# Xiugapurin/Etude

Measured on NVIDIA B200. Metric: extract_throughput_audio_seconds_per_second, higher is better.
Workload: dtype bf16

## Files before the change

etude_b200/csrc/api.cu:

```cuda
#include <algorithm>
#include <cmath>
#include <cstdarg>
#include <cstdio>
#include <cstdlib>
#include <cstring>
#include <string>
#include <map>
#include <vector>

#include "../../include/etude_b200.h"
#include "../../include/etude_b200_kernels.h"
#include "attention2.cuh"
#include "attention4.cuh"
#include "attn_qkv.cuh"
#include "attn_pair.cuh"
#include "chain3.cuh"
#include "embed2.cuh"
#include "gemm.cuh"
#include "logmel.cuh"
#include "logmel2.cuh"
#include "ingest.cuh"
#include "notes.cuh"
#include "pairmma.cuh"
#ifdef ETUDE_DEV_BUILD
// ... 476 lines not shown
    set_smem((const void*)gemm_tcgen05_kernel<256, EPI_BIAS>, gemm_smem_bytes<256, EPI_BIAS>());
    set_smem((const void*)gemm_tcgen05_kernel<256, EPI_BIAS_RELU>, gemm_smem_bytes<256, EPI_BIAS_RELU>());
    set_smem((const void*)gemm_tcgen05_kernel<256, EPI_RESID_LN>, gemm_smem_bytes<256, EPI_RESID_LN>());
#endif
    set_smem((const void*)gemm_tcgen05_kernel<144, EPI_HEADS>, gemm_smem_bytes<144, EPI_HEADS>());
    set_smem((const void*)gemm_bstat_kernel, kGemmBsSmemBytes);
    set_smem((const void*)attention2_kernel<256>, kAttn2SmemBytes);
    set_smem((const void*)attention2_kernel<96>, kAttn2SmemBytes);
    set_smem((const void*)attention4_kernel<128>, kAttn4SmemBytes);
    set_smem((const void*)attention4_kernel<96>, kAttn4SmemBytes);
#ifdef ETUDE_HAVE_ATTN_QKV_CTA1
    set_smem((const void*)attn_qkv_kernel, kAttnQkvSmemBytes);
#endif
    set_smem((const void*)attn_pair_kernel, kAttnPairSmemBytes);
    set_smem((const void*)chain3_kernel<true>, kChain3SmemBytes);
    set_smem((const void*)chain3_kernel<false>, kChain3SmemBytes);
    set_smem((const void*)embed2_kernel, kEmbed2SmemBytes);
    set_smem((const void*)ingest_pcm_kernel, kIngestSmemBudget);
    auto max_smem_carveout = [&](const void* fn) {
        if (e == cudaSuccess) e = cudaFuncSetAttribute(fn, cudaFuncAttributePreferredSharedMemoryCarveout, (int)cudaSharedmemCarveoutMaxShared);
    };
    for (const void* fn : {(const void*)ingest_pcm_kernel, (const void*)notes_transpose_kernel, (const void*)notes_scan_kernel, (const void*)notes_walk_kernel,
                           (const void*)notes_compact_kernel, (const void*)notes_bases_kernel, (const void*)notes_rank_kernel})
        max_smem_carveout(fn);
    set_smem((const void*)logmel2_kernel, kLogmel2SmemBytes);
    if (e != cudaSuccess) status = fail("cudaFuncSetAttribute failed: %s", cudaGetErrorString(e));
    return status;
}

static int num_sms_cached() {
    static int n = 0;
    if (!n) {
        int dev = 0;
        cudaGetDevice(&dev);
        cudaDeviceGetAttribute(&n, cudaDevAttrMultiProcessorCount, dev);
        if (n <= 0) n = 148;
    }
    return n;
}

struct GemmIO {
    __nv_bfloat16* out_bf16 = nullptr;
    int ld_out = 0;
    float* out_f32 = nullptr;
    const float* resid = nullptr;
    int64_t resid_rows = 0;
};

template <int BLOCK_N, int EPI>
static int launch_gemm(const void* a, const void* w, GemmParams p, const GemmIO& io, cudaStream_t st, Profile* prof = nullptr) {
    if (p.K % kBlockK) return fail("gemm: K=%d not a multiple of %d", p.K, kBlockK);
    if (p.N % BLOCK_N) return fail("gemm: N=%d not a multiple of the tile width %d", p.N, BLOCK_N);
    CUtensorMap ta, tb, tob, tof, tr;
    if (make_tmap(&ta, a, (uint64_t)p.M, (uint64_t)p.K, (uint64_t)p.K, kBlockM)) return -1;
    if (make_tmap(&tb, w, (uint64_t)p.N, (uint64_t)p.K, (uint64_t)p.K, BLOCK_N)) return -1;
    tob = ta; tof = ta; tr = ta;
    if (EPI == EPI_BIAS || EPI == EPI_BIAS_RELU) {
        if (!io.out_bf16) return fail("gemm: missing bf16 output");
        if (make_tmap_ex(&tob, io.out_bf16, (uint64_t)p.M, (uint64_t)p.N, (uint64_t)io.ld_out, 32, 64, 2)) return -1;
    } else if (EPI == EPI_RESID_LN) {
        if (!io.out_bf16 || !io.out_f32 || !io.resid) return fail("gemm: LayerNorm epilogue needs out_bf16, out_f32 and resid");
        if (make_tmap_ex(&tob, io.out_bf16, (uint64_t)p.M, 256, 256, 32, 32, 2)) return -1;
        if (make_tmap_ex(&tof, io.out_f32, (uint64_t)p.M, 256, 256, 32, 32, 4)) return -1;
        if (make_tmap_ex(&tr, io.resid, (uint64_t)io.resid_rows, 256, 256, 32, 32, 4)) return -1;
    }
    p.num_m_tiles = (p.M + kBlockM - 1) / kBlockM;
    p.num_n_tiles = p.N / BLOCK_N;
    const int tiles = p.num_m_tiles * p.num_n_tiles;
    const int grid = std::min(tiles, num_sms_cached());
    const int cls = EPI == EPI_RESID_LN ? PC_GEMM_LN : (EPI == EPI_HEADS ? PC_GEMM_HEADS : PC_GEMM_BIAS);
    const int n_alg = EPI == EPI_HEADS ? 3 + kVel : p.N;
    cudaEvent_t ev = prof ? prof->begin(cls, st, 2.0 * p.M * (double)n_alg * p.K, 0.0) : nullptr;
    gemm_tcgen05_kernel<BLOCK_N, EPI><<<grid, kGemmThreads, gemm_smem_bytes<BLOCK_N, EPI>(), st>>>(ta, tb, tob, tof, tr, p);
    if (prof) prof->end(ev, st);
    CUDA_OK(cudaGetLastError());
    {
        char what[96];
        snprintf(what, sizeof what, "gemm epi=%d M=%d N=%d K=%d", EPI, p.M, p.N, p.K);
        if (debug_sync(what, st)) return -1;
    }
    return 0;
}

static int launch_gemm_bstat(const void* a, const void* w, const float* bias, int M, int N, __nv_bfloat16* out, cudaStream_t st, Profile* prof) {
    if (N % 256) return fail("gemm_bstat: N=%d not a multiple of 256", N);
    CUtensorMap ta, tb, to;
    if (make_tmap(&ta, a, (uint64_t)M, 256, 256, kBlockM)) return -1;
    if (make_tmap(&tb, w, (uint64_t)N, 256, 256, 256)) return -1;
    if (make_tmap_ex(&to, out, (uint64_t)M, (uint64_t)N, (uint64_t)N, 32, 64, 2)) return -1;
    GemmParams p{};
    p.M = M; p.N = N; p.K = 256; p.bias = bias;
    p.num_m_tiles = (M + kBlockM - 1) / kBlockM;
    p.num_n_tiles = N / 256;
    const int grid = std::max(1, num_sms_cached() / p.num_n_tiles) * p.num_n_tiles;
    cudaEvent_t ev = prof ? prof->begin(PC_GEMM_BIAS, st, 2.0 * M * (double)N * 256.0, 0.0) : nullptr;
    gemm_bstat_kernel<<<grid, kBsThreads, kGemmBsSmemBytes, st>>>(ta, tb, to, p);
    if (prof) prof->end(ev, st);
    CUDA_OK(cudaGetLastError());
    {
        char what[96];
        snprintf(what, sizeof what, "gemm_bstat M=%d N=%d", M, N);
        if (debug_sync(what, st)) return -1;
    }
    return 0;
}

static int gemm_bias(const void* a, const Linear& L, int M, __nv_bfloat16* out, cudaStream_t st, Profile* prof) {
    if (L.k != 256 || L.n % 256 != 0) return fail("gemm_bias: unsupported projection shape N=%d K=%d", L.n, L.k);
    return launch_gemm_bstat(a, L.w, L.b, M, L.n, out, st, prof);
}

static long long* g_chain_trace = nullptr;

static int launch_attention(const void* q, int64_t q_rows, int q_ld, int q_col0, int q_seq_stride, const void* kv, int kv_ld,
                            int k_col0, int v_col0, int n_seq, int Lq, int Lk, __nv_bfloat16* out, float* probs, cudaStream_t st,
                            Profile* prof = nullptr) {
    const int gen = probs != nullptr ? 2 : 4;
    Attn2Params p{};
    int kb;
    if (Lk == 88) kb = 96;
    else if (Lk == 128) kb = 128;
    else if (Lk == 256 || Lk == 512) kb = gen == 4 ? 128 : 256;
    else return fail("attention: unsupported key length %d", Lk);
    if (Lq > 512 || Lq < 1) return fail("attention: unsupported query length %d", Lq);
    p.Lq = Lq; p.Lk = Lk; p.n_items = n_seq * kHeads; p.q_seq_stride = q_seq_stride;
    p.QT = (Lq + 127) / 128;
    p.NKV = (Lk + kb - 1) / kb;
    if (probs && (p.NKV != 1 || kb == 128)) return fail("attention: the probabilities output is built for one block of 88 or 256 keys");
    if (gen == 4 ? (2 * p.NKV > kA4KvSlots) : (2 * p.NKV + 1 > kA2KvSlots || p.NKV > 2))
        return fail("attention: %d KV blocks exceed the smem ring", p.NKV);
    p.q_col0 = q_col0; p.k_col0 = k_col0; p.v_col0 = v_col0;
    p.out = out; p.probs = probs;
    p.trace = g_chain_trace;
    p.scale_log2e = 1.4426950408889634f / 8.0f;
    CUtensorMap tq, tkv;
    if (make_tmap(&tq, q, (uint64_t)q_rows, (uint64_t)q_ld, (uint64_t)q_ld, 128)) return -1;
    if (make_tmap(&tkv, kv, (uint64_t)n_seq * Lk, (uint64_t)kv_ld, (uint64_t)kv_ld, kb)) return -1;
    const int grid = std::min(p.n_items, num_sms_cached());
    cudaEvent_t ev = prof ? prof->begin(PC_ATTN, st, 4.0 * n_seq * kHeads * (double)Lq * Lk * kHeadDim, 0.0) : nullptr;
    if (gen == 2) {
        if (kb == 256) attention2_kernel<256><<<grid, kAttn2Threads, kAttn2SmemBytes, st>>>(tq, tkv, p);
        else attention2_kernel<96><<<grid, kAttn2Threads, kAttn2SmemBytes, st>>>(tq, tkv, p);
    } else {
        if (kb == 128) attention4_kernel<128><<<grid, kAttn4Threads, kAttn4SmemBytes, st>>>(tq, tkv, p);
        else attention4_kernel<96><<<grid, kAttn4Threads, kAttn4SmemBytes, st>>>(tq, tkv, p);
    }
    if (prof) prof->end(ev, st);
    CUDA_OK(cudaGetLastError());
    {
        char what[96];
        snprintf(what, sizeof what, "attention gen%d n_seq=%d Lq=%d Lk=%d", gen, n_seq, Lq, Lk);
        if (debug_sync(what, st)) return -1;
    }
    return 0;
}

#ifdef ETUDE_DEV_BUILD
extern "C" int etude_debug_mma_bench(int mode, int n, int iters, int n_bufs, int grid, int64_t* host_out) {
    long long* d = nullptr;
    CUDA_OK(cudaMalloc((void**)&d, 16));
    CUDA_OK(cudaFuncSetAttribute((const void*)mma_bench_kernel, cudaFuncAttributeMaxDynamicSharedMemorySize, 210 * 1024));
    mma_bench_kernel<<<grid, 128, 210 * 1024>>>(mode, n, iters, n_bufs, d);
    CUDA_OK(cudaDeviceSynchronize());
    CUDA_OK(cudaMemcpy(host_out, d, 16, cudaMemcpyDeviceToHost));
    cudaFree(d);
    return 0;
}

extern "C" int etude_debug_mma_mix(int ts, int iters, int n_ld, int st_too, int grid, int64_t* host_out) {
    long long* d = nullptr;
    CUDA_OK(cudaMalloc((void**)&d, 32));
    CUDA_OK(cudaMemset(d, 0, 32));
    CUDA_OK(cudaFuncSetAttribute((const void*)mma_mix_kernel, cudaFuncAttributeMaxDynamicSharedMemorySize, 140 * 1024));
    mma_mix_kernel<<<grid, 768, 140 * 1024>>>(ts, iters, n_ld, st_too, d);
    CUDA_OK(cudaDeviceSynchronize());
    CUDA_OK(cudaMemcpy(host_out, d, 16, cudaMemcpyDeviceToHost));
    cudaFree(d);
    return 0;
}

extern "C" int etude_debug_tmem_bench(int mode, int n_warps, int iters, int grid, int64_t* host_out) {
    long long* d = nullptr;
    CUDA_OK(cudaMalloc((void**)&d, 32));
    CUDA_OK(cudaMemset(d, 0, 32));
    tmem_bench_kernel<<<grid, 32 * n_warps>>>(mode, iters, d, reinterpret_cast<float*>(d + 2));
    CUDA_OK(cudaDeviceSynchronize());
    CUDA_OK(cudaMemcpy(host_out, d, 8, cudaMemcpyDeviceToHost));
    cudaFree(d);
    return 0;
}

extern "C" int etude_debug_chain_trace(int enable, int64_t* host_out, int n_values) {
    const size_t bytes = (size_t)64 * 1024;
    if (host_out && g_chain_trace) {
        CUDA_OK(cudaDeviceSynchronize());
// ... 796 lines not shown
```

etude_b200/csrc/attn_qkv.cuh:

```cuda
#pragma once
#include "attention4.cuh"
#include "cluster.cuh"
#include "common.cuh"

namespace etude {

constexpr int kAqThreads = 24 * 32;
constexpr int kAqWStages = 3;
constexpr int kAqXBytes = 4 * 128 * 64 * 2;
constexpr int kAqWStageBytes = 192 * 64 * 2;
constexpr int kAqWHalfBytes = kAqWStageBytes / 2;
constexpr int kAqKVBytes = 2 * 128 * 64 * 2;
constexpr int kAqQBytes = 128 * 64 * 2;
constexpr int kAqStatBytes = 2 * 2 * 2 * 128 * 4;
constexpr size_t kAttnQkvSmemBytes = kAqXBytes + kAqWStages * kAqWStageBytes + 2 * kAqKVBytes + kAqQBytes + kAqStatBytes + 768 * 4 + 512;

#ifndef AQ_W_MULTICAST
#define AQ_W_MULTICAST 1
#endif
#ifndef AQ_COPY_SPLIT
#define AQ_COPY_SPLIT 1
#endif

struct AttnQkvParams {
    int n_seq;
    const float* bias;
    __nv_bfloat16* out;
    float scale_log2e;
    long long* trace;
};

#define AQ_TRACE(role, n, e)                                                                        \
    do {                                                                                            \
        if (p.trace != nullptr && blockIdx.x == 0 && lane == 0 && (n) < 64)                         \
            p.trace[(((role) * 64 + (n)) << 3) + (e)] = clock64();                                  \
    } while (0)

__device__ __forceinline__ void dsmem_bulk_copy(uint32_t dst_cluster_addr, uint32_t src_cta_addr, uint32_t bytes, uint32_t bar_cluster_addr) {
    asm volatile("cp.async.bulk.shared::cluster.shared::cta.mbarrier::complete_tx::bytes [%0], [%1], %2, [%3];" ::"r"(dst_cluster_addr),
                 "r"(src_cta_addr), "r"(bytes), "r"(bar_cluster_addr)
                 : "memory");
}
__device__ __forceinline__ void fence_proxy_async_all() { asm volatile("fence.proxy.async;" ::: "memory"); }
__device__ __forceinline__ void mbar_wait_cl(uint64_t* bar, uint32_t parity) {
    const uint32_t addr = smem_u32(bar);
    auto try_once = [&]() -> bool {
        uint32_t ok;
        asm volatile(
            "{\n\t.reg .pred p;\n\t"
            "mbarrier.try_wait.parity.acquire.cluster.shared::cta.b64 p, [%1], %2;\n\t"
            "selp.u32 %0, 1, 0, p;\n\t}"
            : "=r"(ok)
            : "r"(addr), "r"(parity)
            : "memory");
        return ok != 0;
    };
    if (try_once()) return;
    const unsigned long long t0 = globaltimer_ns();
#pragma unroll 1
    for (;;) {
#pragma unroll 1
        for (uint32_t i = 0; i < 4096u; ++i)
            if (try_once()) return;
        if (globaltimer_ns() - t0 > kWaitBudgetNs) break;
    }
    __trap();
}

#ifndef ETUDE_ATTN_PAIR
#define ETUDE_ATTN_PAIR 1
#endif
#if defined(ETUDE_DEV_BUILD) || !ETUDE_ATTN_PAIR
#define ETUDE_HAVE_ATTN_QKV_CTA1 1
__global__ void __cluster_dims__(2, 1, 1) __launch_bounds__(kAqThreads, 1)
attn_qkv_kernel(const __grid_constant__ CUtensorMap tmap_x, const __grid_constant__ CUtensorMap tmap_w, const AttnQkvParams p) {
    constexpr int O_COL = 192, BUF0_COL = 256, BUF_COLS = 128;
    extern __shared__ __align__(1024) uint8_t smem_raw[];
    uint8_t* smem = smem_raw;
    if ((smem_u32(smem_raw) & 1023u) != 0) __trap();
    uint8_t* sX = smem;
    uint8_t* sW = sX + kAqXBytes;
    uint8_t* sK = sW + kAqWStages * kAqWStageBytes;
    uint8_t* sV = sK + kAqKVBytes;
    uint8_t* sQ = sV + kAqKVBytes;
    float* s_mx = reinterpret_cast<float*>(sQ + kAqQBytes);
    float* s_l = s_mx + 2 * 2 * 128;
    float* s_bias = s_l + 2 * 2 * 128;
    uint64_t* bars = reinterpret_cast<uint64_t*>(s_bias + 768);
    uint64_t* w_full = bars;
    uint64_t* w_empty = w_full + kAqWStages;
    uint64_t* x_full = w_empty + kAqWStages;
    uint64_t* x_free = x_full + 1;
    uint64_t* acc_full = x_free + 1;
    uint64_t* acc_free = acc_full + 1;
    uint64_t* qk_ready = acc_free + 1;
    uint64_t* qk_free = qk_ready + 1;
    uint64_t* v_ready = qk_free + 1;
    uint64_t* v_free = v_ready + 1;
    uint64_t* s_full = v_free + 1;
    uint64_t* p_full = s_full + 2;
    uint64_t* buf_free = p_full + 4;
    uint64_t* o_full = buf_free + 2;
    uint64_t* o_free = o_full + 1;
    uint32_t* tmem_base_ptr = reinterpret_cast<uint32_t*>(o_free + 1);

    const int warp = __shfl_sync(0xffffffffu, threadIdx.x >> 5, 0);
    const int lane = threadIdx.x & 31;
    const uint32_t rank = cluster_ctarank(), peer = rank ^ 1u;
    const int cid = (int)cluster_id_x(), ncl = (int)cluster_nctaid_x();
    const int my_items = (cid < p.n_seq) ? (p.n_seq - 1 - cid) / ncl + 1 : 0;
    const int N = my_items * 4;
    constexpr uint16_t kBoth = 3;

    if (threadIdx.x == 0) {
        tma_prefetch_desc(&tmap_x);
        tma_prefetch_desc(&tmap_w);
        for (int s = 0; s < kAqWStages; ++s) { mbar_init(&w_full[s], 1); mbar_init(&w_empty[s], AQ_W_MULTICAST ? 2 : 1); }
        mbar_init(x_full, 1); mbar_init(x_free, 1);
        mbar_init(acc_full, 1); mbar_init(acc_free, 8);
        mbar_init(qk_ready, 1); mbar_init(qk_free, 2);
        mbar_init(v_ready, 1); mbar_init(v_free, 2);
        for (int b = 0; b < 2; ++b) { mbar_init(&s_full[b], 1); mbar_init(&buf_free[b], 1); }
        for (int b = 0; b < 4; ++b) mbar_init(&p_full[b], 4);
        mbar_init(o_full, 1); mbar_init(o_free, 4);
        mbar_fence_init();
    }
    if (warp == 1) tmem_alloc(tmem_base_ptr, 512);
    for (int i = threadIdx.x; i < 768; i += kAqThreads) s_bias[i] = p.bias[i];
    tc_fence_before();
    __syncthreads();
    cluster_sync_all();
    tc_fence_after();
    const uint32_t tmem_base = *tmem_base_ptr;

    if (warp < 4) {
      reg_dec<40>();
      if (warp == 0) {
        const bool leader = elect_one();
        uint32_t c = 0;
        for (int il = 0; il < my_items; ++il) {
            const int seq = cid + il * ncl;
            const int row0 = seq * 256 + (int)rank * 128;
            mbar_wait_inl(x_free, (il & 1) ^ 1);
            AQ_TRACE(0, il * 4, 0);
            if (leader) {
                mbar_expect_tx(x_full, kAqXBytes);
#pragma unroll
                for (int kc = 0; kc < 4; ++kc) tma_load_2d(sX + kc * 16384, &tmap_x, x_full, kc * 64, row0);
            }
            for (int hk = 0; hk < 16; ++hk, ++c) {
// ... 293 lines not shown
```

etude_b200/csrc/cluster.cuh:

```cuda
#pragma once
#include "common.cuh"

namespace etude {

__device__ __forceinline__ uint32_t cluster_ctarank() {
    uint32_t r;
    asm volatile("mov.u32 %0, %%cluster_ctarank;" : "=r"(r));
    return r;
}
__device__ __forceinline__ uint32_t cluster_id_x() {
    uint32_t r;
    asm volatile("mov.u32 %0, %%clusterid.x;" : "=r"(r));
    return r;
}
__device__ __forceinline__ uint32_t cluster_nctaid_x() {
    uint32_t r;
    asm volatile("mov.u32 %0, %%nclusterid.x;" : "=r"(r));
    return r;
}
__device__ __forceinline__ void cluster_sync_all() {
    asm volatile("barrier.cluster.arrive.release;" ::: "memory");
    asm volatile("barrier.cluster.wait.acquire;" ::: "memory");
}
__device__ __forceinline__ void tma_load_2d_mc(void* smem_dst, const CUtensorMap* m, uint64_t* bar, int c0, int c1, uint16_t mask) {
    asm volatile(
        "cp.async.bulk.tensor.2d.shared::cluster.global.mbarrier::complete_tx::bytes.multicast::cluster [%0], [%1, {%3, %4}], [%2], %5;" ::"r"(
            smem_u32(smem_dst)),
        "l"(reinterpret_cast<uint64_t>(m)), "r"(smem_u32(bar)), "r"(c0), "r"(c1), "h"(mask)
        : "memory");
}
__device__ __forceinline__ void tc_commit_mc(uint64_t* bar, uint16_t mask) {
    asm volatile("tcgen05.commit.cta_group::1.mbarrier::arrive::one.shared::cluster.multicast::cluster.b64 [%0], %1;" ::"r"(smem_u32(bar)),
                 "h"(mask)
                 : "memory");
}

__device__ __forceinline__ uint32_t mapa_u32(uint32_t local_addr, uint32_t rank) {
    uint32_t r;
    asm volatile("mapa.shared::cluster.u32 %0, %1, %2;" : "=r"(r) : "r"(local_addr), "r"(rank));
    return r;
}
__device__ __forceinline__ void mbar_arrive_cluster(uint32_t cluster_addr) {
    asm volatile("mbarrier.arrive.release.cluster.shared::cluster.b64 _, [%0];" ::"r"(cluster_addr) : "memory");
}

__device__ __forceinline__ void mbar_arrive_cluster_relaxed(uint32_t cluster_addr) {
    asm volatile("mbarrier.arrive.relaxed.cluster.shared::cluster.b64 _, [%0];" ::"r"(cluster_addr) : "memory");
}

}
```

etude_b200/csrc/gemm.cuh:

```cuda
#pragma once
#include "common.cuh"

namespace etude {

enum GemmEpilogue : int {
    EPI_BIAS = 0,
    EPI_BIAS_RELU = 1,
    EPI_RESID_LN = 2,
    EPI_HEADS = 3,
};

struct GemmParams {
    int M, N, K;
    int num_m_tiles, num_n_tiles;
    const float* bias;
    int resid_mod;
    const float* ln_gamma;
    const float* ln_beta;
    int heads_time_major;
    const int64_t* heads_row0;
    float* roll_onset;
    float* roll_offset;
    float* roll_mpe;
    int8_t* roll_velocity;
    float* vel_logits;
    int frames;
    int keep0, keepn;
};

constexpr int kGemmThreads = 192;
constexpr int kBlockM = 128;
constexpr int kBlockK = 64;

template <int EPI>
__host__ __device__ constexpr int gemm_stages() { return EPI == EPI_RESID_LN ? 2 : 4; }
template <int EPI>
__host__ __device__ constexpr int gemm_epi_bytes_per_warp() {
    return EPI == EPI_RESID_LN ? (2 * 4096  + 2 * 4096  + 2 * 2048 )
                               : (EPI == EPI_HEADS ? 0 : 2 * 4096 );
}
template <int BLOCK_N, int EPI>
constexpr size_t gemm_smem_bytes() {
    return 1024  + (size_t)gemm_stages<EPI>() * (kBlockM * kBlockK * 2 + BLOCK_N * kBlockK * 2) +
           4 * gemm_epi_bytes_per_warp<EPI>() + (EPI == EPI_RESID_LN ? 3 : 1) * 1024  + 256 ;
}

template <int BLOCK_N, int EPI>
__global__ void __launch_bounds__(kGemmThreads, 1)
gemm_tcgen05_kernel(const __grid_constant__ CUtensorMap tmap_a, const __grid_constant__ CUtensorMap tmap_b,
                    const __grid_constant__ CUtensorMap tmap_out_bf16, const __grid_constant__ CUtensorMap tmap_out_f32,
                    const __grid_constant__ CUtensorMap tmap_resid, const GemmParams p) {
    extern __shared__ uint8_t smem_raw[];
    uint8_t* smem = reinterpret_cast<uint8_t*>((reinterpret_cast<uintptr_t>(smem_raw) + 1023) & ~uintptr_t(1023));
    constexpr int STAGES = gemm_stages<EPI>();
    constexpr int A_BYTES = kBlockM * kBlockK * 2;
    constexpr int B_BYTES = BLOCK_N * kBlockK * 2;
    constexpr int STAGE_BYTES = A_BYTES + B_BYTES;
    constexpr int EPI_BYTES = gemm_epi_bytes_per_warp<EPI>();
    uint8_t* epi_all = smem + STAGES * STAGE_BYTES;
    uint64_t* bars = reinterpret_cast<uint64_t*>(epi_all + 4 * EPI_BYTES);
    float* s_bias = reinterpret_cast<float*>(epi_all + 4 * EPI_BYTES + 256);
    float* s_gamma = s_bias + 256;
    float* s_beta = s_gamma + 256;
    uint64_t* full_bar = bars;
    uint64_t* empty_bar = bars + STAGES;
    uint64_t* tmem_full = bars + 2 * STAGES;
    uint64_t* tmem_empty = bars + 2 * STAGES + 2;
    uint64_t* resid_bar = bars + 2 * STAGES + 4;
    uint32_t* tmem_base_ptr = reinterpret_cast<uint32_t*>(bars + 2 * STAGES + 12);

    const int warp = __shfl_sync(0xffffffffu, threadIdx.x >> 5, 0);
    const int lane = threadIdx.x & 31;
    const int num_tiles = p.num_m_tiles * p.num_n_tiles;
    const int num_kb = p.K / kBlockK;

    if (warp == 0 && lane == 0) {
        tma_prefetch_desc(&tmap_a);
        tma_prefetch_desc(&tmap_b);
        if (EPI != EPI_HEADS) tma_prefetch_desc(&tmap_out_bf16);
        if (EPI == EPI_RESID_LN) {
            tma_prefetch_desc(&tmap_out_f32);
            tma_prefetch_desc(&tmap_resid);
        }
        for (int s = 0; s < STAGES; ++s) {
            mbar_init(&full_bar[s], 1);
            mbar_init(&empty_bar[s], 1);
        }
        for (int s = 0; s < 2; ++s) {
            mbar_init(&tmem_full[s], 1);
            mbar_init(&tmem_empty[s], 4);
        }
        for (int s = 0; s < 8; ++s) mbar_init(&resid_bar[s], 1);
        mbar_fence_init();
    }
    if (warp == 1) tmem_alloc(tmem_base_ptr, 512);
    if (EPI == EPI_RESID_LN && warp >= 2) {
        for (int i = threadIdx.x - 64; i < 256; i += 128) {
            s_bias[i] = p.bias[i];
            s_gamma[i] = p.ln_gamma[i];
            s_beta[i] = p.ln_beta[i];
        }
    }
    tc_fence_before();
    __syncthreads();
    tc_fence_after();
    const uint32_t tmem_base = *tmem_base_ptr;

    if (warp == 0) {
        const bool leader = elect_one();
        int stage = 0;
// ... 174 lines not shown
                        y.y = (v[4 * g + 1] - mean) * rstd * ga.y + be.y;
                        y.z = (v[4 * g + 2] - mean) * rstd * ga.z + be.z;
                        y.w = (v[4 * g + 3] - mean) * rstd * ga.w + be.w;
                        *reinterpret_cast<float4*>(of32 + lane * 128 + ((g ^ (lane & 7)) << 4)) = y;
                        v[4 * g + 0] = y.x; v[4 * g + 1] = y.y; v[4 * g + 2] = y.z; v[4 * g + 3] = y.w;
                    }
#pragma unroll
                    for (int g = 0; g < 4; ++g) {
                        uint4 pk;
                        pk.x = pack_bf16x2(v[8 * g + 0], v[8 * g + 1]); pk.y = pack_bf16x2(v[8 * g + 2], v[8 * g + 3]);
                        pk.z = pack_bf16x2(v[8 * g + 4], v[8 * g + 5]); pk.w = pack_bf16x2(v[8 * g + 6], v[8 * g + 7]);
                        *reinterpret_cast<uint4*>(ob16 + lane * 64 + ((g ^ ((lane >> 1) & 3)) << 4)) = pk;
                    }
                    fence_async_smem();
                    __syncwarp();
                    if (lane == 0) {
                        tma_store_2d(&tmap_out_f32, of32, c * 32, row0);
                        tma_store_2d(&tmap_out_bf16, ob16, c * 32, row0);
                        tma_store_commit();
                    }
                    ++n_store;
                }
            } else {
                const int row = row0 + lane;
                float best = -INFINITY;
                int best_i = 0;
                float head3[3] = {0.f, 0.f, 0.f};
                size_t out_idx = 0, logit_row = 0;
                bool kept = false;
                if (row < p.M) {
                    int w, f, n;
                    if (p.heads_time_major) {
                        f = row % p.frames;
                        const int wn = row / p.frames;
                        n = wn % kNotes;
                        w = wn / kNotes;
                    } else {
                        n = row % kNotes;
                        const int wf = row / kNotes;
                        f = wf % p.frames;
                        w = wf / p.frames;
                    }
                    kept = f >= p.keep0 && f < p.keep0 + p.keepn;
                    out_idx = (size_t)(p.heads_row0[w] + f - p.keep0) * kNotes + n;
                    logit_row = ((size_t)w * p.frames + f) * kNotes + n;
                }
#pragma unroll 1
                for (int c = 0; c < 5; ++c) {
                    tmem_ld32(tbase + c * 32, v);
                    tc_wait_ld();
#pragma unroll
                    for (int j = 0; j < 32; ++j) {
                        const int col = c * 32 + j;
                        if (col < 3 + kVel) {
                            const float x = v[j] + __ldg(&p.bias[col]);
                            if (col < 3) {
                                if (c == 0 && j < 3) head3[j < 3 ? j : 0] = x;
                            } else {
                                if (x > best) { best = x; best_i = col - 3; }
                                if (p.vel_logits && row < p.M) p.vel_logits[logit_row * kVel + (col - 3)] = x;
                            }
                        }
                    }
                }
                if (kept) {
                    p.roll_onset[out_idx] = 1.f / (1.f + expf(-head3[0]));
                    p.roll_offset[out_idx] = 1.f / (1.f + expf(-head3[1]));
                    p.roll_mpe[out_idx] = 1.f / (1.f + expf(-head3[2]));
                    p.roll_velocity[out_idx] = (int8_t)best_i;
                }
            }
            tc_fence_before();
            __syncwarp();
            if (lane == 0) mbar_arrive(&tmem_empty[as]);
            if (++as == 2) { as = 0; aphase ^= 1; }
        }
        if (EPI != EPI_HEADS && lane == 0) tma_store_wait_all<0>();
    }
    tc_fence_before();
    __syncthreads();
    if (warp == 1) tmem_dealloc(tmem_base, 512);
}

constexpr int kBsStages = 4;
constexpr int kBsThreads = 10 * 32;
constexpr int kBsABytes = kBlockM * kBlockK * 2;
constexpr int kBsBBytes = 256 * kBlockK * 2;
constexpr size_t kGemmBsSmemBytes = 4 * kBsBBytes + kBsStages * kBsABytes + 8 * 4096  + 1024  + 256;

__global__ void __launch_bounds__(kBsThreads, 1)
gemm_bstat_kernel(const __grid_constant__ CUtensorMap tmap_a, const __grid_constant__ CUtensorMap tmap_b,
                  const __grid_constant__ CUtensorMap tmap_out, const GemmParams p) {
    extern __shared__ __align__(1024) uint8_t smem_raw[];
    uint8_t* smem = smem_raw;
    if ((smem_u32(smem_raw) & 1023u) != 0) __trap();
    uint8_t* sB = smem;
    uint8_t* sA = sB + 4 * kBsBBytes;
    uint8_t* epi_all = sA + kBsStages * kBsABytes;
    float* s_bias = reinterpret_cast<float*>(epi_all + 8 * 4096);
    uint64_t* bars = reinterpret_cast<uint64_t*>(epi_all + 8 * 4096 + 1024);
    uint64_t* full_bar = bars;
    uint64_t* empty_bar = bars + kBsStages;
    uint64_t* tmem_full = bars + 2 * kBsStages;
    uint64_t* tmem_empty = bars + 2 * kBsStages + 2;
    uint64_t* b_full = bars + 2 * kBsStages + 4;
    uint32_t* tmem_base_ptr = reinterpret_cast<uint32_t*>(bars + 2 * kBsStages + 5);

    const int warp = __shfl_sync(0xffffffffu, threadIdx.x >> 5, 0);
    const int lane = threadIdx.x & 31;
    const int groups = gridDim.x / p.num_n_tiles;
    const int n_blk = blockIdx.x % p.num_n_tiles;
    const int m_first = blockIdx.x / p.num_n_tiles;
    const int col0 = n_blk * 256;

    if (warp == 0 && lane == 0) {
        tma_prefetch_desc(&tmap_a); tma_prefetch_desc(&tmap_b); tma_prefetch_desc(&tmap_out);
        for (int s = 0; s < kBsStages; ++s) { mbar_init(&full_bar[s], 1); mbar_init(&empty_bar[s], 1); }
        for (int s = 0; s < 2; ++s) { mbar_init(&tmem_full[s], 1); mbar_init(&tmem_empty[s], 8); }
        mbar_init(b_full, 1);
        mbar_fence_init();
    }
    if (warp == 1) tmem_alloc(tmem_base_ptr, 512);
    if (warp >= 2)
        for (int i = threadIdx.x - 64; i < 256; i += 256) s_bias[i] = p.bias[col0 + i];
    tc_fence_before();
    __syncthreads();
    tc_fence_after();
    const uint32_t tmem_base = *tmem_base_ptr;

    if (warp == 0) {
        const bool leader = elect_one();
        if (m_first < p.num_m_tiles) {
            if (leader) {
                mbar_expect_tx(b_full, 4 * kBsBBytes);
                for (int kb = 0; kb < 4; ++kb) tma_load_2d(sB + kb * kBsBBytes, &tmap_b, b_full, kb * kBlockK, col0);
            }
            int stage = 0;
            uint32_t phase = 0;
            for (int m_blk = m_first; m_blk < p.num_m_tiles; m_blk += groups)
                for (int kb = 0; kb < 4; ++kb) {
                    mbar_wait(&empty_bar[stage], phase ^ 1);
                    if (leader) {
                        mbar_expect_tx(&full_bar[stage], kBsABytes);
                        tma_load_2d(sA + stage * kBsABytes, &tmap_a, &full_bar[stage], kb * kBlockK, m_blk * kBlockM);
                    }
                    __syncwarp();
                    if (++stage == kBsStages) { stage = 0; phase ^= 1; }
                }
        }
    } else if (warp == 1) {
        const bool leader = elect_one();
        if (m_first < p.num_m_tiles) {
            constexpr uint32_t idesc = make_idesc_bf16(kBlockM, 256, 0, 0);
            const uint64_t a_desc0 = make_sw128_desc(smem_u32(sA)), b_desc0 = make_sw128_desc(smem_u32(sB));
            int stage = 0, as = 0;
            uint32_t phase = 0, aphase = 0;
            mbar_wait(b_full, 0);
            for (int m_blk = m_first; m_blk < p.num_m_tiles; m_blk += groups) {
                mbar_wait(&tmem_empty[as], aphase ^ 1);
                tc_fence_after();
                const uint32_t tmem_d = tmem_base + as * 256;
#pragma unroll
                for (int kb = 0; kb < 4; ++kb) {
                    mbar_wait(&full_bar[stage], phase);
                    tc_fence_after();
                    if (leader) {
                        const uint64_t ad = a_desc0 + (uint64_t)(stage * (kBsABytes >> 4)), bd = b_desc0 + (uint64_t)(kb * (kBsBBytes >> 4));
#pragma unroll
                        for (int k = 0; k < kBlockK / 16; ++k) umma_bf16_ss(tmem_d, ad + 2 * k, bd + 2 * k, idesc, (kb | k) != 0);
                        tc_commit(&empty_bar[stage]);
                    }
                    __syncwarp();
                    if (++stage == kBsStages) { stage = 0; phase ^= 1; }
                }
                if (leader) tc_commit(&tmem_full[as]);
                if (++as == 2) { as = 0; aphase ^= 1; }
            }
        }
    } else {
        const int q = warp & 3, ew = warp - 2, half = ew >> 2;
        uint8_t* obuf = epi_all + ew * 4096;
        int as = 0;
        uint32_t aphase = 0;
        for (int m_blk = m_first; m_blk < p.num_m_tiles; m_blk += groups) {
            const int row0 = m_blk * kBlockM + q * 32;
            mbar_wait(&tmem_full[as], aphase);
            __syncwarp();
            tc_fence_after();
            const uint32_t tbase = tmem_base + as * 256 + ((uint32_t)(q * 32) << 16);
#pragma unroll 1
            for (int c = 2 * half; c < 2 * half + 2; ++c) {
                float v[64];
                tmem_ld32(tbase + c * 64, v);
                tmem_ld32(tbase + c * 64 + 32, v + 32);
                tc_wait_ld();
                uint4 pk[8];
                const float4* b4 = reinterpret_cast<const float4*>(s_bias + c * 64);
#pragma unroll
                for (int g = 0; g < 8; ++g) {
                    const float4 ba = b4[2 * g], bb = b4[2 * g + 1];
                    pk[g].x = pack_bf16x2(v[8 * g + 0] + ba.x, v[8 * g + 1] + ba.y); pk[g].y = pack_bf16x2(v[8 * g + 2] + ba.z, v[8 * g + 3] + ba.w);
                    pk[g].z = pack_bf16x2(v[8 * g + 4] + bb.x, v[8 * g + 5] + bb.y); pk[g].w = pack_bf16x2(v[8 * g + 6] + bb.z, v[8 * g + 7] + bb.w);
                }
                if (c == 2 * half + 1) {
                    tc_fence_before();
                    __syncwarp();
                    if (lane == 0) mbar_arrive(&tmem_empty[as]);
                }
                if (lane == 0) tma_store_wait_read<0>();
                __syncwarp();
#pragma unroll
                for (int g = 0; g < 8; ++g) *reinterpret_cast<uint4*>(obuf + lane * 128 + ((g ^ (lane & 7)) << 4)) = pk[g];
                fence_async_smem();
                __syncwarp();
                if (lane == 0) {
                    tma_store_2d(&tmap_out, obuf, col0 + c * 64, row0);
                    tma_store_commit();
                }
            }
            if (++as == 2) { as = 0; aphase ^= 1; }
        }
        if (lane == 0) tma_store_wait_all<0>();
    }
    tc_fence_before();
    __syncthreads();
    if (warp == 1) tmem_dealloc(tmem_base, 512);
}

__global__ void __launch_bounds__(256)
transpose_time_kernel(const __nv_bfloat16* __restrict__ in, const float* __restrict__ pos_time, float scale, int n_rows, int frames,
                      __nv_bfloat16* __restrict__ out) {
    const int row = blockIdx.x * 8 + (threadIdx.x >> 5);
    if (row >= n_rows) return;
    const int lane = threadIdx.x & 31;
    const int n = row % kNotes, wf = row / kNotes;
    const int f = wf % frames, w = wf / frames;
    const size_t prow = ((size_t)w * kNotes + n) * frames + f;
    const uint4 a = __ldg(reinterpret_cast<const uint4*>(in + (size_t)row * kHid) + lane);
    const float4 p0 = __ldg(reinterpret_cast<const float4*>(pos_time + (size_t)f * kHid) + 2 * lane);
    const float4 p1 = __ldg(reinterpret_cast<const float4*>(pos_time + (size_t)f * kHid) + 2 * lane + 1);
    const uint32_t wv[4] = {a.x, a.y, a.z, a.w};
    float x[8];
#pragma unroll
    for (int i = 0; i < 4; ++i) {
        x[2 * i] = __uint_as_float(wv[i] << 16);
        x[2 * i + 1] = __uint_as_float(wv[i] & 0xFFFF0000u);
    }
    uint4 o;
    o.x = pack_bf16x2(x[0] * scale + p0.x, x[1] * scale + p0.y);
    o.y = pack_bf16x2(x[2] * scale + p0.z, x[3] * scale + p0.w);
    o.z = pack_bf16x2(x[4] * scale + p1.x, x[5] * scale + p1.y);
    o.w = pack_bf16x2(x[6] * scale + p1.z, x[7] * scale + p1.w);
    reinterpret_cast<uint4*>(out + prow * kHid)[lane] = o;
}

__global__ void __launch_bounds__(256) cvt_bf16_to_f32_kernel(const __nv_bfloat16* __restrict__ in, float* __restrict__ out, size_t n8) {
    const size_t i = (size_t)blockIdx.x * 256 + threadIdx.x;
    if (i >= n8) return;
    const uint4 a = __ldg(reinterpret_cast<const uint4*>(in) + i);
    const uint32_t wv[4] = {a.x, a.y, a.z, a.w};
    float4 lo, hi;
    lo.x = __uint_as_float(wv[0] << 16); lo.y = __uint_as_float(wv[0] & 0xFFFF0000u);
    lo.z = __uint_as_float(wv[1] << 16); lo.w = __uint_as_float(wv[1] & 0xFFFF0000u);
    hi.x = __uint_as_float(wv[2] << 16); hi.y = __uint_as_float(wv[2] & 0xFFFF0000u);
    hi.z = __uint_as_float(wv[3] << 16); hi.w = __uint_as_float(wv[3] & 0xFFFF0000u);
    reinterpret_cast<float4*>(out)[2 * i] = lo;
    reinterpret_cast<float4*>(out)[2 * i + 1] = hi;
}
__global__ void __launch_bounds__(256) cvt_f32_to_bf16_kernel(const float* __restrict__ in, __nv_bfloat16* __restrict__ out, size_t n8) {
    const size_t i = (size_t)blockIdx.x * 256 + threadIdx.x;
    if (i >= n8) return;
    const float4 lo = __ldg(reinterpret_cast<const float4*>(in) + 2 * i), hi = __ldg(reinterpret_cast<const float4*>(in) + 2 * i + 1);
    uint4 o;
    o.x = pack_bf16x2(lo.x, lo.y); o.y = pack_bf16x2(lo.z, lo.w); o.z = pack_bf16x2(hi.x, hi.y); o.w = pack_bf16x2(hi.z, hi.w);
    reinterpret_cast<uint4*>(out)[i] = o;
}

}
```

Before: 5790.

## Convert bias GEMM to 2-CTA cluster tcgen05 MMA with split B tile

```diff
diff --git a/etude_b200/csrc/api.cu b/etude_b200/csrc/api.cu
--- a/etude_b200/csrc/api.cu
+++ b/etude_b200/csrc/api.cu
@@ -582,19 +582,22 @@
     return 0;
 }
 
+static long long* g_chain_trace = nullptr;
+
 static int launch_gemm_bstat(const void* a, const void* w, const float* bias, int M, int N, __nv_bfloat16* out, cudaStream_t st, Profile* prof) {
     if (N % 256) return fail("gemm_bstat: N=%d not a multiple of 256", N);
     CUtensorMap ta, tb, to;
     if (make_tmap(&ta, a, (uint64_t)M, 256, 256, kBlockM)) return -1;
-    if (make_tmap(&tb, w, (uint64_t)N, 256, 256, 256)) return -1;
+    if (make_tmap(&tb, w, (uint64_t)N, 256, 256, 128)) return -1;
     if (make_tmap_ex(&to, out, (uint64_t)M, (uint64_t)N, (uint64_t)N, 32, 64, 2)) return -1;
     GemmParams p{};
     p.M = M; p.N = N; p.K = 256; p.bias = bias;
+    p.trace = g_chain_trace;
     p.num_m_tiles = (M + kBlockM - 1) / kBlockM;
     p.num_n_tiles = N / 256;
-    const int grid = std::max(1, num_sms_cached() / p.num_n_tiles) * p.num_n_tiles;
+    const int clusters = std::max(1, num_sms_cached() / 2 / p.num_n_tiles) * p.num_n_tiles;
     cudaEvent_t ev = prof ? prof->begin(PC_GEMM_BIAS, st, 2.0 * M * (double)N * 256.0, 0.0) : nullptr;
-    gemm_bstat_kernel<<<grid, kBsThreads, kGemmBsSmemBytes, st>>>(ta, tb, to, p);
+    gemm_bstat_kernel<<<2 * clusters, kBsThreads, kGemmBsSmemBytes, st>>>(ta, tb, to, p);
     if (prof) prof->end(ev, st);
     CUDA_OK(cudaGetLastError());
     {
@@ -609,8 +612,6 @@
     if (L.k != 256 || L.n % 256 != 0) return fail("gemm_bias: unsupported projection shape N=%d K=%d", L.n, L.k);
     return launch_gemm_bstat(a, L.w, L.b, M, L.n, out, st, prof);
 }
-
-static long long* g_chain_trace = nullptr;
 
 static int launch_attention(const void* q, int64_t q_rows, int q_ld, int q_col0, int q_seq_stride, const void* kv, int kv_ld,
                             int k_col0, int v_col0, int n_seq, int Lq, int Lk, __nv_bfloat16* out, float* probs, cudaStream_t st,
diff --git a/etude_b200/csrc/attn_qkv.cuh b/etude_b200/csrc/attn_qkv.cuh
--- a/etude_b200/csrc/attn_qkv.cuh
+++ b/etude_b200/csrc/attn_qkv.cuh
@@ -42,30 +42,6 @@
                  : "memory");
 }
 __device__ __forceinline__ void fence_proxy_async_all() { asm volatile("fence.proxy.async;" ::: "memory"); }
-__device__ __forceinline__ void mbar_wait_cl(uint64_t* bar, uint32_t parity) {
-    const uint32_t addr = smem_u32(bar);
-    auto try_once = [&]() -> bool {
-        uint32_t ok;
-        asm volatile(
-            "{\n\t.reg .pred p;\n\t"
-            "mbarrier.try_wait.parity.acquire.cluster.shared::cta.b64 p, [%1], %2;\n\t"
-            "selp.u32 %0, 1, 0, p;\n\t}"
-            : "=r"(ok)
-            : "r"(addr), "r"(parity)
-            : "memory");
-        return ok != 0;
-    };
-    if (try_once()) return;
-    const unsigned long long t0 = globaltimer_ns();
-#pragma unroll 1
-    for (;;) {
-#pragma unroll 1
-        for (uint32_t i = 0; i < 4096u; ++i)
-            if (try_once()) return;
-        if (globaltimer_ns() - t0 > kWaitBudgetNs) break;
-    }
-    __trap();
-}
 
 #ifndef ETUDE_ATTN_PAIR
 #define ETUDE_ATTN_PAIR 1
diff --git a/etude_b200/csrc/cluster.cuh b/etude_b200/csrc/cluster.cuh
--- a/etude_b200/csrc/cluster.cuh
+++ b/etude_b200/csrc/cluster.cuh
@@ -48,4 +48,29 @@
     asm volatile("mbarrier.arrive.relaxed.cluster.shared::cluster.b64 _, [%0];" ::"r"(cluster_addr) : "memory");
 }
 
+__device__ __forceinline__ void mbar_wait_cl(uint64_t* bar, uint32_t parity) {
+    const uint32_t addr = smem_u32(bar);
+    auto try_once = [&]() -> bool {
+        uint32_t ok;
+        asm volatile(
+            "{\n\t.reg .pred p;\n\t"
+            "mbarrier.try_wait.parity.acquire.cluster.shared::cta.b64 p, [%1], %2;\n\t"
+            "selp.u32 %0, 1, 0, p;\n\t}"
+            : "=r"(ok)
+            : "r"(addr), "r"(parity)
+            : "memory");
+        return ok != 0;
+    };
+    if (try_once()) return;
+    const unsigned long long t0 = globaltimer_ns();
+#pragma unroll 1
+    for (;;) {
+#pragma unroll 1
+        for (uint32_t i = 0; i < 4096u; ++i)
+            if (try_once()) return;
+        if (globaltimer_ns() - t0 > kWaitBudgetNs) break;
+    }
+    __trap();
 }
+
+}
diff --git a/etude_b200/csrc/gemm.cuh b/etude_b200/csrc/gemm.cuh
--- a/etude_b200/csrc/gemm.cuh
+++ b/etude_b200/csrc/gemm.cuh
@@ -1,5 +1,6 @@
 #pragma once
 #include "common.cuh"
+#include "pairmma.cuh"
 
 namespace etude {
 
@@ -26,6 +27,7 @@
     float* vel_logits;
     int frames;
     int keep0, keepn;
+    long long* trace;
 };
 
 constexpr int kGemmThreads = 192;
@@ -366,13 +368,25 @@
     if (warp == 1) tmem_dealloc(tmem_base, 512);
 }
 
-constexpr int kBsStages = 4;
+constexpr int kBsStages = 6;
+constexpr int kBsBoxes = 2;
 constexpr int kBsThreads = 10 * 32;
 constexpr int kBsABytes = kBlockM * kBlockK * 2;
-constexpr int kBsBBytes = 256 * kBlockK * 2;
-constexpr size_t kGemmBsSmemBytes = 4 * kBsBBytes + kBsStages * kBsABytes + 8 * 4096  + 1024  + 256;
-
-__global__ void __launch_bounds__(kBsThreads, 1)
+constexpr int kBsBBytes = 128 * kBlockK * 2;
+constexpr size_t kGemmBsSmemBytes = 4 * kBsBBytes + kBsStages * kBsABytes + 8 * kBsBoxes * 4096  + 1024  + 256;
+
+constexpr int kBsTrTile0 = 16, kBsTrTiles = 64;
+#ifdef ETUDE_DEV_BUILD
+#define BS_TRACE(role, it, e)                                                                                              \
+    do {                                                                                                                   \
+        if (p.trace != nullptr && tr_cta && lane == 0 && (it) >= kBsTrTile0 && (it) < kBsTrTile0 + kBsTrTiles)              \
+            p.trace[((((int)rank * 4 + (role)) * kBsTrTiles + (it) - kBsTrTile0) << 3) + (e)] = clock64() - t_origin + 1;   \
+    } while (0)
+#else
+#define BS_TRACE(role, it, e) do { } while (0)
+#endif
+
+__global__ void __cluster_dims__(2, 1, 1) __launch_bounds__(kBsThreads, 1)
 gemm_bstat_kernel(const __grid_constant__ CUtensorMap tmap_a, const __grid_constant__ CUtensorMap tmap_b,
                   const __grid_constant__ CUtensorMap tmap_out, const GemmParams p) {
     extern __shared__ __align__(1024) uint8_t smem_raw[];
@@ -381,8 +395,8 @@
     uint8_t* sB = smem;
     uint8_t* sA = sB + 4 * kBsBBytes;
     uint8_t* epi_all = sA + kBsStages * kBsABytes;
-    float* s_bias = reinterpret_cast<float*>(epi_all + 8 * 4096);
-    uint64_t* bars = reinterpret_cast<uint64_t*>(epi_all + 8 * 4096 + 1024);
+    float* s_bias = reinterpret_cast<float*>(epi_all + 8 * kBsBoxes * 4096);
+    uint64_t* bars = reinterpret_cast<uint64_t*>(epi_all + 8 * kBsBoxes * 4096 + 1024);
     uint64_t* full_bar = bars;
     uint64_t* empty_bar = bars + kBsStages;
     uint64_t* tmem_full = bars + 2 * kBsStages;
@@ -392,85 +406,105 @@
 
     const int warp = __shfl_sync(0xffffffffu, threadIdx.x >> 5, 0);
     const int lane = threadIdx.x & 31;
-    const int groups = gridDim.x / p.num_n_tiles;
-    const int n_blk = blockIdx.x % p.num_n_tiles;
-    const int m_first = blockIdx.x / p.num_n_tiles;
+    const uint32_t rank = cluster_ctarank();
+    const bool lead_cta = rank == 0;
+    const int cid = (int)cluster_id_x();
+    const int groups = (int)cluster_nctaid_x() / p.num_n_tiles;
+    const int n_blk = cid % p.num_n_tiles;
+    const int pair_first = cid / p.num_n_tiles;
+    const int num_pairs = (p.num_m_tiles + 1) / 2;
     const int col0 = n_blk * 256;
 
-    if (warp == 0 && lane == 0) {
+    if (threadIdx.x == 0) {
         tma_prefetch_desc(&tmap_a); tma_prefetch_desc(&tmap_b); tma_prefetch_desc(&tmap_out);
         for (int s = 0; s < kBsStages; ++s) { mbar_init(&full_bar[s], 1); mbar_init(&empty_bar[s], 1); }
-        for (int s = 0; s < 2; ++s) { mbar_init(&tmem_full[s], 1); mbar_init(&tmem_empty[s], 8); }
+        for (int s = 0; s < 2; ++s) { mbar_init(&tmem_full[s], 1); mbar_init(&tmem_empty[s], 16); }
         mbar_init(b_full, 1);
         mbar_fence_init();
     }
-    if (warp == 1) tmem_alloc(tmem_base_ptr, 512);
+    if (warp == 1) tmem_alloc2(tmem_base_ptr, 512);
     if (warp >= 2)
         for (int i = threadIdx.x - 64; i < 256; i += 256) s_bias[i] = p.bias[col0 + i];
     tc_fence_before();
     __syncthreads();
+    cluster_sync_all();
     tc_fence_after();
     const uint32_t tmem_base = *tmem_base_ptr;
+    const bool tr_cta = cid == 0;
+    const long long t_origin = clock64();
+    (void)tr_cta; (void)t_origin;
 
     if (warp == 0) {
         const bool leader = elect_one();
-        if (m_first < p.num_m_tiles) {
+        if (pair_first < num_pairs) {
             if (leader) {
-                mbar_expect_tx(b_full, 4 * kBsBBytes);
-                for (int kb = 0; kb < 4; ++kb) tma_load_2d(sB + kb * kBsBBytes, &tmap_b, b_full, kb * kBlockK, col0);
-            }
-            int stage = 0;
+                if (lead_cta) mbar_expect_tx(b_full, 2 * 4 * kBsBBytes);
+                const uint32_t b_full_l = mapa_u32(smem_u32(b_full), 0);
+                for (int kb = 0; kb < 4; ++kb) tma_load_2d_pair(sB + kb * kBsBBytes, &tmap_b, b_full_l, kb * kBlockK, col0 + (int)rank * 128);
+            }
+            const uint32_t full_l0 = mapa_u32(smem_u32(full_bar), 0);
+            int stage = 0, it = 0;
             uint32_t phase = 0;
-            for (int m_blk = m_first; m_blk < p.num_m_tiles; m_blk += groups)
+            for (int pr = pair_first; pr < num_pairs; pr += groups, ++it) {
+                const int m_blk = 2 * pr + (int)rank;
                 for (int kb = 0; kb < 4; ++kb) {
-                    mbar_wait(&empty_bar[stage], phase ^ 1);
+                    mbar_wait_cl(&empty_bar[stage], phase ^ 1);
+                    BS_TRACE(0, it, kb);
                     if (leader) {
-                        mbar_expect_tx(&full_bar[stage], kBsABytes);
-                        tma_load_2d(sA + stage * kBsABytes, &tmap_a, &full_bar[stage], kb * kBlockK, m_blk * kBlockM);
+                        if (lead_cta) mbar_expect_tx(&full_bar[stage], 2 * kBsABytes);
+                        tma_load_2d_pair(sA + stage * kBsABytes, &tmap_a, full_l0 + stage * 8, kb * kBlockK, m_blk * kBlockM);
                     }
                     __syncwarp();
                     if (++stage == kBsStages) { stage = 0; phase ^= 1; }
                 }
+            }
         }
     } else if (warp == 1) {
         const bool leader = elect_one();
-        if (m_first < p.num_m_tiles) {
-            constexpr uint32_t idesc = make_idesc_bf16(kBlockM, 256, 0, 0);
+        if (lead_cta && pair_first < num_pairs) {
+            constexpr uint32_t idesc = make_idesc_bf16(2 * kBlockM, 256, 0, 0);
             const uint64_t a_desc0 = make_sw128_desc(smem_u32(sA)), b_desc0 = make_sw128_desc(smem_u32(sB));
-            int stage = 0, as = 0;
+            int stage = 0, as = 0, it = 0;
             uint32_t phase = 0, aphase = 0;
-            mbar_wait(b_full, 0);
-            for (int m_blk = m_first; m_blk < p.num_m_tiles; m_blk += groups) {
-                mbar_wait(&tmem_empty[as], aphase ^ 1);
+            mbar_wait_cl(b_full, 0);
+            for (int pr = pair_first; pr < num_pairs; pr += groups, ++it) {
+                mbar_wait_cl(&tmem_empty[as], aphase ^ 1);
                 tc_fence_after();
+                BS_TRACE(1, it, 0);
                 const uint32_t tmem_d = tmem_base + as * 256;
 #pragma unroll
                 for (int kb = 0; kb < 4; ++kb) {
-                    mbar_wait(&full_bar[stage], phase);
+                    mbar_wait_cl(&full_bar[stage], phase);
                     tc_fence_after();
+                    BS_TRACE(1, it, 1 + kb);
                     if (leader) {
                         const uint64_t ad = a_desc0 + (uint64_t)(stage * (kBsABytes >> 4)), bd = b_desc0 + (uint64_t)(kb * (kBsBBytes >> 4));
 #pragma unroll
-                        for (int k = 0; k < kBlockK / 16; ++k) umma_bf16_ss(tmem_d, ad + 2 * k, bd + 2 * k, idesc, (kb | k) != 0);
-                        tc_commit(&empty_bar[stage]);
+                        for (int k = 0; k < kBlockK / 16; ++k) umma2_bf16_ss(tmem_d, ad + 2 * k, bd + 2 * k, idesc, (kb | k) != 0);
+                        tc_commit2_mc(&empty_bar[stage], 3);
                     }
                     __syncwarp();
                     if (++stage == kBsStages) { stage = 0; phase ^= 1; }
                 }
-                if (leader) tc_commit(&tmem_full[as]);
+                if (leader) tc_commit2_mc(&tmem_full[as], 3);
+                BS_TRACE(1, it, 5);
                 if (++as == 2) { as = 0; aphase ^= 1; }
             }
         }
     } else {
         const int q = warp & 3, ew = warp - 2, half = ew >> 2;
-        uint8_t* obuf = epi_all + ew * 4096;
-        int as = 0;
+        uint8_t* obuf0 = epi_all + ew * kBsBoxes * 4096;
+        const int tr_role = (ew & 3) == 0 ? 2 + half : 4;
+        (void)tr_role;
+        const uint32_t tmem_empty_l0 = mapa_u32(smem_u32(tmem_empty), 0);
+        int as = 0, it = 0;
         uint32_t aphase = 0;
-        for (int m_blk = m_first; m_blk < p.num_m_tiles; m_blk += groups) {
-            const int row0 = m_blk * kBlockM + q * 32;
-            mbar_wait(&tmem_full[as], aphase);
+        for (int pr = pair_first; pr < num_pairs; pr += groups, ++it) {
+            const int row0 = (2 * pr + (int)rank) * kBlockM + q * 32;
+            mbar_wait_cl(&tmem_full[as], aphase);
             __syncwarp();
             tc_fence_after();
+            if (tr_role < 4) BS_TRACE(tr_role, it, 0);
             const uint32_t tbase = tmem_base + as * 256 + ((uint32_t)(q * 32) << 16);
 #pragma unroll 1
             for (int c = 2 * half; c < 2 * half + 2; ++c) {
@@ -478,6 +512,7 @@
                 tmem_ld32(tbase + c * 64, v);
                 tmem_ld32(tbase + c * 64 + 32, v + 32);
                 tc_wait_ld();
+                if (tr_role < 4) BS_TRACE(tr_role, it, 1 + 3 * (c & 1));
                 uint4 pk[8];
                 const float4* b4 = reinterpret_cast<const float4*>(s_bias + c * 64);
 #pragma unroll
@@ -489,10 +524,15 @@
                 if (c == 2 * half + 1) {
                     tc_fence_before();
                     __syncwarp();
-                    if (lane == 0) mbar_arrive(&tmem_empty[as]);
-                }
-                if (lane == 0) tma_store_wait_read<0>();
+                    if (lane == 0) {
+                        if (lead_cta) mbar_arrive(&tmem_empty[as]);
+                        else mbar_arrive_cluster_relaxed(tmem_empty_l0 + as * 8);
+                    }
+                }
+                uint8_t* obuf = obuf0 + (c & 1) * 4096;
+                if (lane == 0) tma_store_wait_read<kBsBoxes - 1>();
                 __syncwarp();
+                if (tr_role < 4) BS_TRACE(tr_role, it, 2 + 3 * (c & 1));
 #pragma unroll
                 for (int g = 0; g < 8; ++g) *reinterpret_cast<uint4*>(obuf + lane * 128 + ((g ^ (lane & 7)) << 4)) = pk[g];
                 fence_async_smem();
@@ -501,6 +541,7 @@
                     tma_store_2d(&tmap_out, obuf, col0 + c * 64, row0);
                     tma_store_commit();
                 }
+                if (tr_role < 4) BS_TRACE(tr_role, it, 3 + 3 * (c & 1));
             }
             if (++as == 2) { as = 0; aphase ^= 1; }
         }
@@ -508,7 +549,8 @@
     }
     tc_fence_before();
     __syncthreads();
-    if (warp == 1) tmem_dealloc(tmem_base, 512);
+    cluster_sync_all();
+    if (warp == 1) tmem_dealloc2(tmem_base, 512);
 }
 
 __global__ void __launch_bounds__(256)
```

Result: no change. 5833 (median of 6 runs) (+0.8%).
